# Ascend-Research/HeadPoseEstimation-WHENet

Measured on NVIDIA H100. Metric: head-crops/sec @224x224 bf16, higher is better.
Workload: dtype bf16

## Files before the change

headposeestimation-whenet_b200/build.py:

```python
from __future__ import annotations

import os
import subprocess
import sys

HERE = os.path.dirname(os.path.abspath(__file__))
CSRC = os.path.join(HERE, "csrc")
OBJ = os.path.join(CSRC, "obj")
LIB = os.path.join(HERE, "libwhenet_b200.so")
_SIMT_TC = ["kernels_simt.cuh", "kernels_tc.cuh"]
_ABI = os.path.join("..", "..", "include", "whenet_b200.h")
UNITS = {
    "whenet_api.cu": _SIMT_TC + ["api_error.h", "kernels_fused.cuh", "kernels_crop.cuh", "kernels_overlay.cuh", "hershey_simplex.inc", "yuv.cuh", "kernels_k2.cuh", "kernels_tc32.cuh", "kernels_dwse.cuh", "kernels_k1x.cuh", "jpeg_api.h", _ABI],
    "inst_k1_bf16.cu": _SIMT_TC + ["kernels_fused.cuh", "kernels_dwse.cuh", "kernels_k1x.cuh"],
    "inst_k1_f16.cu": _SIMT_TC + ["kernels_fused.cuh"],
    "inst_dwse.cu": _SIMT_TC + ["kernels_fused.cuh", "kernels_dwse.cuh"],
    "inst_pw.cu": _SIMT_TC + ["kernels_fused.cuh", "kernels_k2.cuh"],
    "inst_yolo.cu": _SIMT_TC + ["kernels_yolo.cuh", "yuv.cuh"],
    "inst_yolo32.cu": _SIMT_TC + ["kernels_yolo.cuh", "kernels_yolo32.cuh", "yuv.cuh"],
    "yolo_api.cu": _SIMT_TC + ["kernels_yolo.cuh", "kernels_yolo32.cuh", "yuv.cuh", "api_error.h", _ABI],
    "jpeg_api.cu": ["kernels_jpeg.cuh", "jpeg_api.h", "api_error.h", _ABI],
}
SOURCES = list(UNITS)
HEADERS = sorted({h for hs in UNITS.values() for h in hs})

NVCC_FLAGS = ["-O3", "-std=c++17", "-gencode", "arch=compute_90a,code=sm_90a", "-lineinfo", "-Xcompiler", "-fPIC,-ffp-contract=off"]


def _obj(src: str) -> str:
    return os.path.join(OBJ, os.path.splitext(src)[0] + ".o")


def _unit_stale(src: str) -> bool:
    o = _obj(src)
    if not os.path.exists(o):
        return True
    t = os.path.getmtime(o)
    deps = [os.path.join(CSRC, d) for d in [src] + UNITS[src]] + [os.path.abspath(__file__)]
    return any(os.path.exists(d) and os.path.getmtime(d) > t for d in deps)


def _stale() -> bool:
    if not os.path.exists(LIB):
        return True
    t = os.path.getmtime(LIB)
    deps = [os.path.join(CSRC, d) for d in SOURCES + HEADERS] + [os.path.abspath(__file__)]
    return any(os.path.exists(d) and os.path.getmtime(d) > t for d in deps)


def build_lib(force: bool = False, verbose: bool = False) -> str:
    if not force and not _stale():
        return LIB
    from concurrent.futures import ThreadPoolExecutor
    nvcc = os.environ.get("NVCC", "/usr/local/cuda/bin/nvcc")
    os.makedirs(OBJ, exist_ok=True)
    todo = [s for s in SOURCES if force or _unit_stale(s)]

    def compile_unit(src):
        cmd = [nvcc] + NVCC_FLAGS + (["-Xptxas=-v"] if verbose else []) + ["-c", "-o", _obj(src), os.path.join(CSRC, src)]
        if verbose:
            print(" ".join(cmd), file=sys.stderr)
        return src, subprocess.run(cmd, capture_output=True, text=True)

    with ThreadPoolExecutor(max_workers=max(1, min(len(todo), os.cpu_count() or 1))) as ex:
        results = list(ex.map(compile_unit, todo))
    for src, r in results:
        if r.returncode != 0:
            raise RuntimeError("nvcc failed on %s:\n%s\n%s" % (src, r.stdout, r.stderr))
        if verbose:
            print(r.stderr, file=sys.stderr)
# ... 10 lines not shown
```

headposeestimation-whenet_b200/csrc/inst_pw.cu:

```cuda
#include "kernels_simt.cuh"
#include "kernels_tc.cuh"
#include "kernels_k2.cuh"

namespace whenet {
namespace tc {
#define WHENET_INST_PW(T)                                                                                                    \
    template int launch_pw_tc2<T>(cudaStream_t, const T*, const void*, const float*, const float*, const T*, T*, long long, \
                                  int, int, int, bool, int, int, int, bool);                                                 \
    template int launch_k2<T>(cudaStream_t, const K2Params&, size_t, bool, bool, bool, int);                \
    template int launch_pw_tc3<T>(cudaStream_t, const T*, const void*, const float*, const float*, const T*, T*, long long, int, int, int);
WHENET_INST_PW(__nv_bfloat16)
WHENET_INST_PW(__half)
#undef WHENET_INST_PW
}
}
```

headposeestimation-whenet_b200/csrc/kernels_tc.cuh:

```cuda
#pragma once
#include <cuda.h>
#include <cuda_bf16.h>
#include <cuda_fp16.h>
#include <cuda_runtime.h>
#include <stdint.h>

#include "kernels_simt.cuh"

namespace whenet {
namespace tc {


constexpr int BM = 128;
constexpr int BK = 64;
constexpr int A_STAGE_BYTES = BM * BK * 2;
constexpr int kAccPitch = 132;
__host__ __device__ constexpr uint32_t acc_tile_bytes(int cols) { return (uint32_t)cols * kAccPitch * 4u; }

__device__ __forceinline__ uint32_t smem_u32(const void* p) { return (uint32_t)__cvta_generic_to_shared(p); }

__device__ __forceinline__ void mbar_init(uint64_t* bar, uint32_t count) {
    asm volatile("mbarrier.init.shared::cta.b64 [%0], %1;" ::"r"(smem_u32(bar)), "r"(count) : "memory");
}
__device__ __forceinline__ bool mbar_wait(uint64_t* bar, uint32_t parity, int* tflag) {
// ... 43 lines not shown
    if ((threadIdx.x & 31) == 0) arrive(bar_addr);
}
__device__ __forceinline__ void arrive_expect_tx(uint32_t bar_addr, uint32_t bytes) {
    asm volatile("mbarrier.arrive.expect_tx.shared::cta.b64 _, [%0], %1;" ::"r"(bar_addr), "r"(bytes) : "memory");
}
__device__ __forceinline__ void tma_4d(uint32_t dst, const CUtensorMap* tm, int c0, int c1, int c2, int c3, uint32_t bar_addr) {
    asm volatile("cp.async.bulk.tensor.4d.shared::cluster.global.mbarrier::complete_tx::bytes [%0], [%1, {%2, %3, %4, %5}], [%6];"
                 ::"r"(dst), "l"(tm), "r"(c0), "r"(c1), "r"(c2), "r"(c3), "r"(bar_addr) : "memory");
}
__device__ __forceinline__ void tma_2d(uint32_t dst, const CUtensorMap* tm, int c0, int c1, uint32_t bar_addr) {
    asm volatile("cp.async.bulk.tensor.2d.shared::cluster.global.mbarrier::complete_tx::bytes [%0], [%1, {%2, %3}], [%4];"
                 ::"r"(dst), "l"(tm), "r"(c0), "r"(c1), "r"(bar_addr) : "memory");
}

}

__device__ __forceinline__ uint64_t make_desc(uint32_t saddr) {
    uint64_t d = 0;
    d |= (uint64_t)((saddr >> 4) & 0x3FFF);
    d |= (uint64_t)1 << 16;
    d |= (uint64_t)64 << 32;
    d |= (uint64_t)1 << 62;
    return d;
}
__device__ __forceinline__ uint64_t make_desc_sw64(uint32_t saddr) {
    uint64_t d = 0;
    d |= (uint64_t)((saddr >> 4) & 0x3FFF);
    d |= (uint64_t)1 << 16;
    d |= (uint64_t)32 << 32;
    d |= (uint64_t)2 << 62;
    return d;
}
template <int ROWB>
__device__ __forceinline__ uint64_t make_desc_rows(uint32_t saddr) {
    static_assert(ROWB == 64 || ROWB == 128, "rows of 64 or 128 bytes");
    if constexpr (ROWB == 64) return make_desc_sw64(saddr);
    else return make_desc(saddr);
}

__device__ __forceinline__ void wg_fence() { asm volatile("wgmma.fence.sync.aligned;" ::: "memory"); }
__device__ __forceinline__ void wg_commit() { asm volatile("wgmma.commit_group.sync.aligned;" ::: "memory"); }
template <int N> __device__ __forceinline__ void wg_wait() { asm volatile("wgmma.wait_group.sync.aligned %0;" ::"n"(N) : "memory"); }

#define WG_D8(g) "+f"(d[8 * g]), "+f"(d[8 * g + 1]), "+f"(d[8 * g + 2]), "+f"(d[8 * g + 3]), \
                 "+f"(d[8 * g + 4]), "+f"(d[8 * g + 5]), "+f"(d[8 * g + 6]), "+f"(d[8 * g + 7])
#define WG_OPS_1 WG_D8(0)
#define WG_OPS_2 WG_OPS_1, WG_D8(1)
#define WG_OPS_3 WG_OPS_2, WG_D8(2)
#define WG_OPS_4 WG_OPS_3, WG_D8(3)
#define WG_OPS_5 WG_OPS_4, WG_D8(4)
#define WG_OPS_6 WG_OPS_5, WG_D8(5)
#define WG_OPS_7 WG_OPS_6, WG_D8(6)
#define WG_OPS_8 WG_OPS_7, WG_D8(7)
#define WG_REGS_1 "%0,%1,%2,%3,%4,%5,%6,%7"
#define WG_REGS_2 WG_REGS_1 ",%8,%9,%10,%11,%12,%13,%14,%15"
#define WG_REGS_3 WG_REGS_2 ",%16,%17,%18,%19,%20,%21,%22,%23"
#define WG_REGS_4 WG_REGS_3 ",%24,%25,%26,%27,%28,%29,%30,%31"
#define WG_REGS_5 WG_REGS_4 ",%32,%33,%34,%35,%36,%37,%38,%39"
#define WG_REGS_6 WG_REGS_5 ",%40,%41,%42,%43,%44,%45,%46,%47"
#define WG_REGS_7 WG_REGS_6 ",%48,%49,%50,%51,%52,%53,%54,%55"
#define WG_REGS_8 WG_REGS_7 ",%56,%57,%58,%59,%60,%61,%62,%63"
#define WG_TAIL_1 "16", "%8, %9", "%10"
#define WG_TAIL_2 "32", "%16, %17", "%18"
#define WG_TAIL_3 "48", "%24, %25", "%26"
#define WG_TAIL_4 "64", "%32, %33", "%34"
#define WG_TAIL_5 "80", "%40, %41", "%42"
#define WG_TAIL_6 "96", "%48, %49", "%50"
#define WG_TAIL_7 "112", "%56, %57", "%58"
#define WG_TAIL_8 "128", "%64, %65", "%66"
#define WG_ASM_(TY, REGS, NS, AB, SC, ...)                                                                              \
    asm volatile("{\n\t.reg .pred p;\n\tsetp.ne.b32 p, " SC ", 0;\n\t"                                                    \
                 "wgmma.mma_async.sync.aligned.m64n" NS "k16.f32." TY "." TY " {" REGS "}, " AB ", p, 1, 1, 0, 0;\n\t}" \
                 : __VA_ARGS__ : "l"(ad), "l"(bd), "r"(accumulate))
#define WG_ASM(TY, REGS, TAIL, OPS) WG_ASM_(TY, REGS, TAIL, OPS)
#define WG_CASE(k)                                                                                                 \
    if constexpr (N == 16 * k) {                                                                                   \
        if constexpr (BF16) WG_ASM("bf16", WG_REGS_##k, WG_TAIL_##k, WG_OPS_##k);                                  \
        else WG_ASM("f16", WG_REGS_##k, WG_TAIL_##k, WG_OPS_##k);                                                  \
    }

template <bool BF16, int N>
__device__ __forceinline__ void wgmma(float (&d)[N / 2], uint64_t ad, uint64_t bd, uint32_t accumulate) {
    static_assert(N % 16 == 0 && N >= 16 && N <= 128, "wgmma: N = 16, 32, ..., 128");
    WG_CASE(1) WG_CASE(2) WG_CASE(3) WG_CASE(4) WG_CASE(5) WG_CASE(6) WG_CASE(7) WG_CASE(8)
}
#undef WG_CASE
#undef WG_ASM
#undef WG_ASM_

template <int N> struct WgAcc { float d[2][N / 2]; };

template <bool BF16, int N, int H, int KS>
__device__ __forceinline__ void wg_mma_run(float (&d)[H][N / 2], uint64_t a0, uint64_t a1, uint64_t b0, uint32_t accumulate) {
    wg_fence();
#pragma unroll
    for (int k = 0; k < KS; ++k) {
        const uint32_t sc = (accumulate | (uint32_t)k) ? 1u : 0u;
        wgmma<BF16, N>(d[0], a0 + (uint64_t)(k * 2), b0 + (uint64_t)(k * 2), sc);
        if constexpr (H == 2) wgmma<BF16, N>(d[1], a1 + (uint64_t)(k * 2), b0 + (uint64_t)(k * 2), sc);
    }
    wg_commit();
}
template <bool BF16, int N, int H>
__device__ __forceinline__ void wg_mma_block(float (&d)[H][N / 2], uint64_t a0, uint64_t a1, uint64_t b0, int ksteps, uint32_t accumulate) {
    if (ksteps >= 4) wg_mma_run<BF16, N, H, 4>(d, a0, a1, b0, accumulate);
    else if (ksteps == 3) wg_mma_run<BF16, N, H, 3>(d, a0, a1, b0, accumulate);
    else if (ksteps == 2) wg_mma_run<BF16, N, H, 2>(d, a0, a1, b0, accumulate);
    else wg_mma_run<BF16, N, H, 1>(d, a0, a1, b0, accumulate);
}

template <bool BF16, int N>
__device__ __forceinline__ void wg_mma_tile(WgAcc<N>& acc, uint32_t a_st, uint32_t b_st, int ksteps, uint32_t accumulate) {
    wg_mma_block<BF16, N, 2>(acc.d, make_desc(a_st), make_desc(a_st + 64 * 128), make_desc(b_st), ksteps, accumulate);
}

template <bool BF16, int N>
__device__ __forceinline__ void wg_mma_m64(float (&d)[N / 2], uint32_t a_st, uint32_t a_kb, uint32_t b_st, uint32_t b_kb, int ksteps) {
    float (&d1)[1][N / 2] = *reinterpret_cast<float(*)[1][N / 2]>(&d);
    for (int kb = 0; kb * 4 < ksteps; ++kb)
        wg_mma_block<BF16, N, 1>(d1, make_desc(a_st + (uint32_t)kb * a_kb), 0, make_desc(b_st + (uint32_t)kb * b_kb), ksteps - 4 * kb, kb ? 1u : 0u);
}

template <int N>
__device__ __forceinline__ void wg_acc_store(const WgAcc<N>& acc, uint32_t dst, int wt) {
    const int w = wt >> 5, l = wt & 31;
    const int r = 16 * w + (l >> 2), cq = 2 * (l & 3);
#pragma unroll
    for (int h = 0; h < 2; ++h)
#pragma unroll
        for (int i = 0; i < N / 8; ++i)
#pragma unroll
            for (int e = 0; e < 4; ++e) {
                const int row = 64 * h + r + (e >> 1) * 8, col = 8 * i + cq + (e & 1);
                asm volatile("st.shared.f32 [%0], %1;" ::"r"(dst + (uint32_t)(col * kAccPitch + row) * 4u), "f"(acc.d[h][4 * i + e]) : "memory");
            }
}

// ... 24 lines not shown
        case 16: return call_with_width<16, MAXW>(f);
        case 32: return call_with_width<32, MAXW>(f);
        case 48: return call_with_width<48, MAXW>(f);
        case 64: return call_with_width<64, MAXW>(f);
        case 96: return call_with_width<96, MAXW>(f);
        case 128: return call_with_width<128, MAXW>(f);
    }
    return 1;
}

__device__ __forceinline__ void acc_ld16(uint32_t base, int row, int c0, float (&v)[16]) {
#pragma unroll
    for (int i = 0; i < 16; ++i)
        asm volatile("ld.shared.f32 %0, [%1];" : "=f"(v[i]) : "r"(base + (uint32_t)((c0 + i) * kAccPitch + row) * 4u));
}

template <typename T> __device__ __forceinline__ uint4 scale8(uint4 raw, const float* g);
template <> __device__ __forceinline__ uint4 scale8<__nv_bfloat16>(uint4 raw, const float* g) {
    __nv_bfloat162* h = reinterpret_cast<__nv_bfloat162*>(&raw);
    const float4 g0 = *reinterpret_cast<const float4*>(g), g1 = *reinterpret_cast<const float4*>(g + 4);
    const float gg[8] = {g0.x, g0.y, g0.z, g0.w, g1.x, g1.y, g1.z, g1.w};
#pragma unroll
    for (int i = 0; i < 4; ++i) {
        float2 f = __bfloat1622float2(h[i]);
        h[i] = __floats2bfloat162_rn(f.x * gg[2 * i], f.y * gg[2 * i + 1]);
    }
    return raw;
}
template <> __device__ __forceinline__ uint4 scale8<__half>(uint4 raw, const float* g) {
    __half2* h = reinterpret_cast<__half2*>(&raw);
    const float4 g0 = *reinterpret_cast<const float4*>(g), g1 = *reinterpret_cast<const float4*>(g + 4);
    const float gg[8] = {g0.x, g0.y, g0.z, g0.w, g1.x, g1.y, g1.z, g1.w};
#pragma unroll
    for (int i = 0; i < 4; ++i) {
        float2 f = __half22float2(h[i]);
        h[i] = __floats2half2_rn(f.x * gg[2 * i], f.y * gg[2 * i + 1]);
    }
    return raw;
}

__device__ __forceinline__ int fdiv_small(int x, float inv) { return __float2int_rz(((float)x + 0.5f) * inv); }
__device__ __forceinline__ void cp_async16_z(uint32_t dst, const void* src, bool valid) {
    const uint32_t sz = valid ? 16u : 0u;
    asm volatile("cp.async.cg.shared.global [%0], [%1], 16, %2;" ::"r"(dst), "l"(src), "r"(sz) : "memory");
}
__device__ __forceinline__ uint4 lds128(uint32_t addr) {
    uint4 v;
    asm volatile("ld.shared.v4.b32 {%0,%1,%2,%3}, [%4];" : "=r"(v.x), "=r"(v.y), "=r"(v.z), "=r"(v.w) : "r"(addr));
    return v;
}
__device__ __forceinline__ void sts128_(uint32_t addr, const uint4& v) {
    asm volatile("st.shared.v4.b32 [%0], {%1,%2,%3,%4};" ::"r"(addr), "r"(v.x), "r"(v.y), "r"(v.z), "r"(v.w) : "memory");
}
template <typename T> __device__ __forceinline__ uint4 scale8s(uint4 raw, uint32_t gaddr);
template <> __device__ __forceinline__ uint4 scale8s<__nv_bfloat16>(uint4 raw, uint32_t gaddr) {
    float4 g0, g1;
    asm volatile("ld.shared.v4.f32 {%0,%1,%2,%3}, [%4];" : "=f"(g0.x), "=f"(g0.y), "=f"(g0.z), "=f"(g0.w) : "r"(gaddr));
    asm volatile("ld.shared.v4.f32 {%0,%1,%2,%3}, [%4];" : "=f"(g1.x), "=f"(g1.y), "=f"(g1.z), "=f"(g1.w) : "r"(gaddr + 16));
    __nv_bfloat162* h = reinterpret_cast<__nv_bfloat162*>(&raw);
    const float gg[8] = {g0.x, g0.y, g0.z, g0.w, g1.x, g1.y, g1.z, g1.w};
#pragma unroll
    for (int i = 0; i < 4; ++i) {
        float2 f = __bfloat1622float2(h[i]);
        h[i] = __floats2bfloat162_rn(f.x * gg[2 * i], f.y * gg[2 * i + 1]);
    }
    return raw;
}
template <> __device__ __forceinline__ uint4 scale8s<__half>(uint4 raw, uint32_t gaddr) {
    float4 g0, g1;
    asm volatile("ld.shared.v4.f32 {%0,%1,%2,%3}, [%4];" : "=f"(g0.x), "=f"(g0.y), "=f"(g0.z), "=f"(g0.w) : "r"(gaddr));
    asm volatile("ld.shared.v4.f32 {%0,%1,%2,%3}, [%4];" : "=f"(g1.x), "=f"(g1.y), "=f"(g1.z), "=f"(g1.w) : "r"(gaddr + 16));
    __half2* h = reinterpret_cast<__half2*>(&raw);
    const float gg[8] = {g0.x, g0.y, g0.z, g0.w, g1.x, g1.y, g1.z, g1.w};
#pragma unroll
    for (int i = 0; i < 4; ++i) {
        float2 f = __half22float2(h[i]);
        h[i] = __floats2half2_rn(f.x * gg[2 * i], f.y * gg[2 * i + 1]);
    }
    return raw;
}

template <typename T, bool SWISH, int GATE, bool RESID, bool OUT_H, int UN>
__global__ void __launch_bounds__(128) pw_tc2_kernel(const T* __restrict__ A, const T* __restrict__ Wt,
                                                     const float* __restrict__ bias, const float* __restrict__ gate,
                                                     const T* __restrict__ resid, T* __restrict__ out,
                                                     int M, int K, int N, int hw,
                                                     int n_tile, int n_stages,
                                                     int tiles_per_crop) {
    constexpr bool BF16 = std::is_same<T, __nv_bfloat16>::value;
    extern __shared__ uint8_t smem_raw[];

    const int tid = threadIdx.x;
    const uint32_t smem0 = (smem_u32(smem_raw) + 1023u) & ~1023u;
    constexpr int w_stage_bytes = UN * BK * 2;
    const uint32_t stage_bytes = A_STAGE_BYTES + w_stage_bytes;
    const uint32_t sG = smem0 + n_stages * stage_bytes;

    int m0, rows_valid, crop0;
    if (GATE == 2) {
        const int crop = blockIdx.y / tiles_per_crop, t = blockIdx.y - crop * tiles_per_crop;
        m0 = crop * hw + t * BM;
        rows_valid = min(BM, hw - t * BM);
        crop0 = crop;
    } else {
        m0 = blockIdx.y * BM;
        rows_valid = min(BM, M - m0);
        crop0 = GATE ? m0 / hw : 0;
    }
    const int n0 = blockIdx.x * n_tile;
    const int n_valid = min(n_tile, N - n0);
    const int nkb = (K + BK - 1) / BK;
    const int kchunks = K >> 3;

    if (GATE) {
        const int ncrops = GATE == 2 ? 1 : ((m0 + rows_valid - 1) / hw - crop0 + 1);
        const int q = K >> 2;
        for (int idx = tid; idx < ncrops * q; idx += 128) {
            const int cr = idx / q, j = idx - cr * q;
            cp_async16_z(sG + (uint32_t)(cr * K + j * 4) * 4, gate + (long long)(crop0 + cr) * K + j * 4, true);
        }
    }
    auto fill = [&](int kb) {
        const int s = kb % n_stages;
        const uint32_t a_st = smem0 + s * stage_bytes, w_st = a_st + A_STAGE_BYTES;
        const int kc0 = kb * 8;
        const int cb = min(8, kchunks - kc0), cbp = (cb + 1) & ~1;
        if (cbp == 8) {
            const int c = tid & 7, r0 = tid >> 3;
            const bool cvalid = c < cb;
            const T* asrc = A + (long long)(m0 + r0) * K + (kc0 + c) * 8;
            const uint32_t swz = (uint32_t)((r0 >> 3) * 1024 + (r0 & 7) * 128 + ((c ^ (r0 & 7)) << 4));
#pragma unroll
// ... 371 lines not shown
```

headposeestimation-whenet_b200/csrc/whenet_api.cu:

```cuda
#include <cuda_bf16.h>
#include <cuda_fp16.h>
#include <cuda_runtime.h>

#include <algorithm>
#include <array>
#include <charconv>
#include <atomic>
#include <cmath>
#include <cstdarg>
#include <cstdio>
#include <cstdlib>
#include <cstring>
#include <map>
#include <string>
#include <thread>
#include <type_traits>
#include <vector>

#include "../../include/whenet_b200.h"
#include "api_error.h"
#include "kernels_simt.cuh"
#include "kernels_tc.cuh"
#include "kernels_fused.cuh"
#include "kernels_crop.cuh"
#include "kernels_overlay.cuh"
#include "kernels_k2.cuh"
#include "kernels_tc32.cuh"
#include "kernels_dwse.cuh"
#include "kernels_k1x.cuh"
#include "jpeg_api.h"
#include <cudaTypedefs.h>

namespace whenet {
namespace fused {
#define WHENET_EXTERN_FUSED(T)                                                                            \
    extern template int launch_k1<T>(cudaStream_t, K1Params, int, int, int, int, size_t, int);            \
    extern template int launch_dw_only<T>(cudaStream_t, K1Params, size_t, int);
WHENET_EXTERN_FUSED(__nv_bfloat16)
WHENET_EXTERN_FUSED(__half)
#undef WHENET_EXTERN_FUSED
extern template int launch_dwse<__nv_bfloat16>(cudaStream_t, DwSeParams, int, int, int, int, int);
extern template int launch_dwse_x<__nv_bfloat16>(cudaStream_t, DwSeParams, int, int, int, int, int);
extern template int launch_dwse_spatial<__nv_bfloat16>(cudaStream_t, DwSeParams, int, int, int);
extern template int launch_k1x<__nv_bfloat16>(cudaStream_t, DwSeParams, int, int, int, int, int, int, int, int);
}
namespace tc {
#define WHENET_EXTERN_PW(T)                                                                                                         \
    extern template int launch_pw_tc2<T>(cudaStream_t, const T*, const void*, const float*, const float*, const T*, T*, long long, \
                                         int, int, int, bool, int, int, int, bool);                                                 \
    extern template int launch_k2<T>(cudaStream_t, const K2Params&, size_t, bool, bool, bool, int);          \
    extern template int launch_pw_tc3<T>(cudaStream_t, const T*, const void*, const float*, const float*, const T*, T*, long long, int, int, int);
WHENET_EXTERN_PW(__nv_bfloat16)
WHENET_EXTERN_PW(__half)
#undef WHENET_EXTERN_PW
}
}

namespace {

using whenet::api::fail;
using whenet::api::g_err;

#define CK(call)                                                                                   \
    do {                                                                                           \
        cudaError_t e__ = (call);                                                                  \
        if (e__ != cudaSuccess)                                                                    \
            return fail(WHENET_ECUDA, "%s failed at %s:%d: %s", #call, __FILE__, __LINE__,         \
                        cudaGetErrorString(e__));                                                  \
    } while (0)

constexpr double kBnEps = 1e-3;
constexpr int kImgElems = 224 * 224 * 3;

struct BlockCfg {
    int idx, hin, hout, cin, cexp, cout, k, s, cse, pad;
    bool skip, has_expand;
};

std::vector<BlockCfg> make_blocks() {
// ... 307 lines not shown

int make_tmap_kd_e(CUtensorMap* tm, const void* base, int n, int H, int C, int cc, int pw) {
    auto fn = tmap_encode_fn();
    if (!fn) return fail(WHENET_ECUDA, "cuTensorMapEncodeTiled is not available from this driver");
    const cuuint64_t dims[4] = {(cuuint64_t)C, (cuuint64_t)H, (cuuint64_t)H, (cuuint64_t)n};
    const cuuint64_t strides[3] = {(cuuint64_t)C * 2, (cuuint64_t)H * C * 2, (cuuint64_t)H * H * C * 2};
    const cuuint32_t box[4] = {(cuuint32_t)cc, (cuuint32_t)pw, (cuuint32_t)pw, 1};
    const cuuint32_t estr[4] = {1, 1, 1, 1};
    const CUresult r = fn(tm, CU_TENSOR_MAP_DATA_TYPE_FLOAT16, 4, const_cast<void*>(base), dims, strides, box, estr, CU_TENSOR_MAP_INTERLEAVE_NONE,
                          CU_TENSOR_MAP_SWIZZLE_NONE, CU_TENSOR_MAP_L2_PROMOTION_L2_128B, CU_TENSOR_MAP_FLOAT_OOB_FILL_NONE);
    if (r != CUDA_SUCCESS) return fail(WHENET_ECUDA, "cuTensorMapEncodeTiled(KD tile %dx%dx%dx%d, box %dx%dx%d) failed: %d", n, H, H, C, pw, pw, cc, (int)r);
    return 0;
}
int make_tmap_k1x_in(CUtensorMap* tm, const void* base, int n, int H, int C, int iw, int row_bytes) {
    auto fn = tmap_encode_fn();
    if (!fn) return fail(WHENET_ECUDA, "cuTensorMapEncodeTiled is not available from this driver");
    const cuuint64_t dims[4] = {(cuuint64_t)C, (cuuint64_t)H, (cuuint64_t)H, (cuuint64_t)n};
    const cuuint64_t strides[3] = {(cuuint64_t)C * 2, (cuuint64_t)H * C * 2, (cuuint64_t)H * H * C * 2};
    const cuuint32_t box[4] = {(cuuint32_t)row_bytes / 2, (cuuint32_t)iw, (cuuint32_t)iw, 1};
    const cuuint32_t estr[4] = {1, 1, 1, 1};
    const CUresult r = fn(tm, CU_TENSOR_MAP_DATA_TYPE_BFLOAT16, 4, const_cast<void*>(base), dims, strides, box, estr, CU_TENSOR_MAP_INTERLEAVE_NONE,
                          row_bytes == 64 ? CU_TENSOR_MAP_SWIZZLE_64B : CU_TENSOR_MAP_SWIZZLE_128B, CU_TENSOR_MAP_L2_PROMOTION_L2_128B,
                          CU_TENSOR_MAP_FLOAT_OOB_FILL_NONE);
    if (r != CUDA_SUCCESS) return fail(WHENET_ECUDA, "cuTensorMapEncodeTiled(K1X input %dx%dx%dx%d, box %dx%d) failed: %d", n, H, H, C, iw, iw, (int)r);
    return 0;
}
int make_tmap_kd_w(CUtensorMap* tm, const void* base, int kk, int C, int cc) {
    auto fn = tmap_encode_fn();
    if (!fn) return fail(WHENET_ECUDA, "cuTensorMapEncodeTiled is not available from this driver");
    const cuuint64_t dims[2] = {(cuuint64_t)C, (cuuint64_t)kk};
    const cuuint64_t strides[1] = {(cuuint64_t)C * 2};
    const cuuint32_t box[2] = {(cuuint32_t)cc, (cuuint32_t)kk};
    const cuuint32_t estr[2] = {1, 1};
    const CUresult r = fn(tm, CU_TENSOR_MAP_DATA_TYPE_FLOAT16, 2, const_cast<void*>(base), dims, strides, box, estr, CU_TENSOR_MAP_INTERLEAVE_NONE,
                          CU_TENSOR_MAP_SWIZZLE_NONE, CU_TENSOR_MAP_L2_PROMOTION_L2_128B, CU_TENSOR_MAP_FLOAT_OOB_FILL_NONE);
    if (r != CUDA_SUCCESS) return fail(WHENET_ECUDA, "cuTensorMapEncodeTiled(KD weights %dx%d, box %d) failed: %d", kk, C, cc, (int)r);
    return 0;
}

template <typename T>
int launch_pw(whenet_ctx* c, const char* name, const T* A, const float* W, const void* Wt16, const float* bias,
              const float* gate, const T* resid, T* out, long long M, int K, int N, int hw, bool swish, bool out_half = false) {
    const double bytes = (double)M * (K + N + (resid ? N : 0)) * sizeof(T);
    const double flops = 2.0 * (double)M * K * N;
    Scope sc(c, name, bytes, flops);
    if constexpr (sizeof(T) == 2) {
        const bool want_k2 = c->pw_variant == 3 || (c->pw_variant == 4 && (gate == nullptr || hw <= 196));
        if (c->use_tc && Wt16 && want_k2 && !out_half) {
            whenet::tc::K2Params kp{};
            size_t smem = 0;
            if (whenet::tc::plan_k2(M, K, N, hw, gate != nullptr, c->precision == WHENET_PRECISION_BF16, &kp, &smem) &&
                (c->pw_variant == 3 || kp.tiles >= 2 * c->sm_count)) {
                if (c->tmaps2.size() > 1024) c->tmaps2.clear();
                const TmapKey ka{K, (int)M, (const void*)A}, kw{-N, K, Wt16};
                auto ia = c->tmaps2.find(ka);
                if (ia == c->tmaps2.end()) {
                    CUtensorMap tm;
                    int rc = make_tmap_w(&tm, A, (int)M, K, whenet::tc::BM, c->precision == WHENET_PRECISION_BF16);
                    if (rc) return rc;
                    ia = c->tmaps2.emplace(ka, tm).first;
                }
                auto iw = c->tmaps2.find(kw);
                if (iw == c->tmaps2.end()) {
                    CUtensorMap tm;
                    int rc = make_tmap_w(&tm, Wt16, N, K, kp.n_tile, c->precision == WHENET_PRECISION_BF16);
                    if (rc) return rc;
                    iw = c->tmaps2.emplace(kw, tm).first;
                }
                kp.tmA = ia->second; kp.tmW = iw->second;
                kp.bias = bias; kp.gate = gate; kp.resid = resid; kp.out = out; kp.tflag = c->d_tflag;
                int rc = whenet::tc::launch_k2<T>(c->stream, kp, smem, swish, gate != nullptr, resid != nullptr, c->sm_count);
                if (rc == 0) { CK(cudaGetLastError()); return 0; }
                if (rc < 0) return fail(WHENET_ECUDA, "K2 launch failed for %s (rc=%d)", name, rc);
            }
        }
        if (c->use_tc && Wt16 && gate && hw >= 784 && c->pw3 && !out_half && !swish) {
            int rc = whenet::tc::launch_pw_tc3<T>(c->stream, A, Wt16, bias, gate, resid, out, M, K, N, hw);
            if (rc == 0) { CK(cudaGetLastError()); return 0; }
            if (rc < 0) return fail(WHENET_ECUDA, "pw_tc3 launch failed for %s (rc=%d)", name, rc);
        }
        if (c->use_tc && Wt16) {
            int rc = whenet::tc::launch_pw_tc2<T>(c->stream, A, Wt16, bias, gate, resid, out, M, K, N, hw, swish, c->pw_stage_cap, c->pw_smem_kb, c->pw_min_ctas, out_half);
            if (rc == 0) { CK(cudaGetLastError()); return 0; }
            if (rc < 0) return fail(WHENET_ECUDA, "tensor-core 1x1 launch failed for %s (rc=%d)", name, rc);
        }
    }
    if constexpr (sizeof(T) == 4) {
        if (c->use_tc && Wt16 && c->split_lo_bytes) {
            int rc = whenet::tc::launch_pw_tc32(c->stream, A, Wt16, (const char*)Wt16 + c->split_lo_bytes, bias, gate, resid, out, M, K, N, hw, swish);
            if (rc == 0) { CK(cudaGetLastError()); return 0; }
            if (rc < 0) return fail(WHENET_ECUDA, "split-bf16 tensor-core 1x1 launch failed for %s (rc=%d)", name, rc);
        }
    }
    if (out_half) return fail(WHENET_EINVAL, "fp16-output 1x1 conv needs the tensor-core kernel (%s)", name);
    dim3 grid((unsigned)((M + 63) / 64), (unsigned)((N + 63) / 64));
#define PW(SW, GA, RE) whenet::pw_conv_kernel<T, SW, GA, RE><<<grid, 256, 0, c->stream>>>(A, W, bias, gate, resid, out, M, K, N, hw)
    if (swish && !gate && !resid) PW(true, false, false);
    else if (!swish && gate && !resid) PW(false, true, false);
    else if (!swish && gate && resid) PW(false, true, true);
    else if (!swish && !gate && !resid) PW(false, false, false);
    else if (!swish && !gate && resid) PW(false, false, true);
    else return fail(WHENET_EINVAL, "unsupported 1x1 epilogue combination");
#undef PW
    CK(cudaGetLastError());
    return 0;
}
// ... 1883 lines not shown
```

Measured before the change: 87470.

## Add crop-pair warp-specialized GEMM for gated 7x7 pointwise layers

Adds a persistent, warp-specialized wgmma kernel for bf16 pointwise convolutions at 7x7 spatial size (49 rows per crop) with N of 192 or 320. Each CTA processes two crops per tile so that TMA-loaded 49-row A tiles line up with crop boundaries. Gating warps apply the SE gate in shared memory between load and MMA, and the epilogue adds bias and optional residual through a shared-memory staging buffer. The wgmma helper is extended to N=160. The aim is to avoid wasted M padding and to fuse the gate scaling into the GEMM pipeline for the late network layers, at the cost of a new code path and a smaller M tile (98 rows) per CTA.

```diff
diff --git a/headposeestimation-whenet_b200/build.py b/headposeestimation-whenet_b200/build.py
--- a/headposeestimation-whenet_b200/build.py
+++ b/headposeestimation-whenet_b200/build.py
@@ -11,11 +11,11 @@
 _SIMT_TC = ["kernels_simt.cuh", "kernels_tc.cuh"]
 _ABI = os.path.join("..", "..", "include", "whenet_b200.h")
 UNITS = {
-    "whenet_api.cu": _SIMT_TC + ["api_error.h", "kernels_fused.cuh", "kernels_crop.cuh", "kernels_overlay.cuh", "hershey_simplex.inc", "yuv.cuh", "kernels_k2.cuh", "kernels_tc32.cuh", "kernels_dwse.cuh", "kernels_k1x.cuh", "jpeg_api.h", _ABI],
+    "whenet_api.cu": _SIMT_TC + ["api_error.h", "kernels_fused.cuh", "kernels_crop.cuh", "kernels_overlay.cuh", "hershey_simplex.inc", "yuv.cuh", "kernels_k2.cuh", "kernels_kp7.cuh", "kernels_tc32.cuh", "kernels_dwse.cuh", "kernels_k1x.cuh", "jpeg_api.h", _ABI],
     "inst_k1_bf16.cu": _SIMT_TC + ["kernels_fused.cuh", "kernels_dwse.cuh", "kernels_k1x.cuh"],
     "inst_k1_f16.cu": _SIMT_TC + ["kernels_fused.cuh"],
     "inst_dwse.cu": _SIMT_TC + ["kernels_fused.cuh", "kernels_dwse.cuh"],
-    "inst_pw.cu": _SIMT_TC + ["kernels_fused.cuh", "kernels_k2.cuh"],
+    "inst_pw.cu": _SIMT_TC + ["kernels_fused.cuh", "kernels_k2.cuh", "kernels_kp7.cuh"],
     "inst_yolo.cu": _SIMT_TC + ["kernels_yolo.cuh", "yuv.cuh"],
     "inst_yolo32.cu": _SIMT_TC + ["kernels_yolo.cuh", "kernels_yolo32.cuh", "yuv.cuh"],
     "yolo_api.cu": _SIMT_TC + ["kernels_yolo.cuh", "kernels_yolo32.cuh", "yuv.cuh", "api_error.h", _ABI],
diff --git a/headposeestimation-whenet_b200/csrc/inst_pw.cu b/headposeestimation-whenet_b200/csrc/inst_pw.cu
--- a/headposeestimation-whenet_b200/csrc/inst_pw.cu
+++ b/headposeestimation-whenet_b200/csrc/inst_pw.cu
@@ -1,6 +1,7 @@
 #include "kernels_simt.cuh"
 #include "kernels_tc.cuh"
 #include "kernels_k2.cuh"
+#include "kernels_kp7.cuh"
 
 namespace whenet {
 namespace tc {
@@ -12,5 +13,21 @@
 WHENET_INST_PW(__nv_bfloat16)
 WHENET_INST_PW(__half)
 #undef WHENET_INST_PW
+
+int launch_kp7(cudaStream_t stream, const KP7Params& p, size_t smem, bool resid) {
+    auto go = [&](auto kfn, int nt) {
+        if (cudaFuncSetAttribute(kfn, cudaFuncAttributeMaxDynamicSharedMemorySize, 225 * 1024) != cudaSuccess) return -1;
+        int dev = 0, sms = 0, per_sm = 0;
+        if (cudaGetDevice(&dev) != cudaSuccess || cudaDeviceGetAttribute(&sms, cudaDevAttrMultiProcessorCount, dev) != cudaSuccess ||
+            cudaOccupancyMaxActiveBlocksPerMultiprocessor(&per_sm, kfn, nt, smem) != cudaSuccess || per_sm < 1)
+            return -1;
+        kfn<<<(unsigned)std::min(p.pairs, per_sm * sms), nt, smem, stream>>>(p);
+        return 0;
+    };
+    if (p.N == 192 && resid) return go(kp7_kernel<192, true>, Kp7<192, true>::NT);
+    if (p.N == 192) return go(kp7_kernel<192, false>, Kp7<192, false>::NT);
+    if (p.N == 320 && !resid) return go(kp7_kernel<320, false>, Kp7<320, false>::NT);
+    return 1;
 }
 }
+}
diff --git a/headposeestimation-whenet_b200/csrc/kernels_kp7.cuh b/headposeestimation-whenet_b200/csrc/kernels_kp7.cuh
--- /dev/null
+++ b/headposeestimation-whenet_b200/csrc/kernels_kp7.cuh
@@ -0,0 +1,244 @@
+#pragma once
+#include <cuda.h>
+
+#include "kernels_fused.cuh"
+
+namespace whenet {
+namespace tc {
+
+constexpr int kKp7Hw = 49;
+constexpr uint32_t kKp7Half = 64 * 128;
+constexpr int kKp7GateThreads = 96;
+constexpr int kKp7MaxStages = 8;
+
+struct alignas(64) KP7Params {
+    CUtensorMap tmA;
+    CUtensorMap tmW;
+    const float* bias;
+    const float* gate;
+    const void* resid;
+    void* out;
+    int* tflag;
+    int K, N, crops, pairs;
+    int nkb, ksteps_last;
+    int stages;
+    uint32_t stage_bytes;
+    uint32_t off_g, off_b, off_o;
+};
+
+template <int N> struct Kp7Geom;
+template <> struct Kp7Geom<192> { static constexpr int NWG = 2, NW = 96; };
+template <> struct Kp7Geom<320> { static constexpr int NWG = 2, NW = 160; };
+
+template <int N, bool RESID>
+struct Kp7 {
+    static constexpr int NWG = Kp7Geom<N>::NWG, NW = Kp7Geom<N>::NW;
+    static constexpr int NT = 128 * (1 + NWG);
+    static constexpr int REG_LAUNCH = (65536 / NT) & ~7;
+    static constexpr int REG_LOW = 72;
+    static constexpr int REG_MMA = ((NT * REG_LAUNCH - 128 * REG_LOW) / (128 * NWG)) & ~7;
+    static constexpr uint32_t PITCH = RESID ? (uint32_t)(NW + 8) * 4u : (uint32_t)NW * 2u + 16u;
+    static constexpr uint32_t WARP_STAGE = 16u * PITCH;
+    static constexpr uint32_t OUT_STAGE = (uint32_t)(4 * NWG) * WARP_STAGE;
+    static_assert(NW % 16 == 0 && NW <= 160 && NW * NWG == N, "MMA width");
+    static_assert(REG_MMA >= NW + 24, "accumulator registers");
+};
+
+template <int N, bool RESID>
+__global__ void __launch_bounds__(Kp7<N, RESID>::NT, 1) kp7_kernel(const __grid_constant__ KP7Params p) {
+    using namespace whenet::fused;
+    using G = Kp7<N, RESID>;
+    constexpr int NW = G::NW;
+    extern __shared__ uint8_t smem_raw[];
+    __shared__ __align__(8) uint64_t bars[3 * kKp7MaxStages];
+    __shared__ int s_abort_mem;
+    volatile int* s_abort = &s_abort_mem;
+
+    const int tid = threadIdx.x, warp = tid >> 5, lane = tid & 31;
+    const uint32_t smem0 = (smem_u32(smem_raw) + 1023u) & ~1023u;
+    const uint32_t sRing = smem0, sG = smem0 + p.off_g, sB = smem0 + p.off_b;
+    const uint32_t bar0 = smem_u32(&bars[0]);
+    const uint32_t b_full = bar0, b_ready = bar0 + 8 * kKp7MaxStages, b_empty = bar0 + 16 * kKp7MaxStages;
+
+    if (tid == 0) {
+        for (int i = 0; i < kKp7MaxStages; ++i) {
+            mbar_init(&bars[i], 1);
+            mbar_init(&bars[kKp7MaxStages + i], kKp7GateThreads / 32);
+            mbar_init(&bars[2 * kKp7MaxStages + i], G::NWG);
+        }
+        s_abort_mem = 0;
+        asm volatile("fence.mbarrier_init.release.cluster;" ::: "memory");
+    }
+    for (int i = tid; i < N; i += G::NT) {
+        const float b = __ldg(p.bias + i);
+        asm volatile("st.shared.f32 [%0], %1;" ::"r"(sB + (uint32_t)i * 4u), "f"(b) : "memory");
+    }
+    __syncthreads();
+
+    const int first = blockIdx.x, step = gridDim.x;
+
+    if (warp < 4) {
+        asm volatile("setmaxnreg.dec.sync.aligned.u32 %0;" ::"n"(G::REG_LOW));
+        if (warp == 0) {
+            if (lane == 0) {
+                asm volatile("prefetch.tensormap [%0];" ::"l"(&p.tmA) : "memory");
+                asm volatile("prefetch.tensormap [%0];" ::"l"(&p.tmW) : "memory");
+                const uint32_t a_bytes = kKp7Hw * 128;
+                int g = 0;
+                for (int pair = first; pair < p.pairs; pair += step) {
+                    const bool two = 2 * pair + 1 < p.crops;
+                    const int row0 = 2 * pair * kKp7Hw;
+                    for (int kb = 0; kb < p.nkb; ++kb, ++g) {
+                        const int s = g % p.stages;
+                        const uint32_t par = (uint32_t)(g / p.stages) & 1u;
+                        mbar::wait(b_empty + 8 * s, par ^ 1, s_abort, p.tflag);
+                        const uint32_t st = sRing + (uint32_t)s * p.stage_bytes;
+                        mbar::arrive_expect_tx(b_full + 8 * s, (two ? 2 : 1) * a_bytes + (uint32_t)N * 128);
+                        mbar::tma_2d(st, &p.tmA, kb * 64, row0, b_full + 8 * s);
+                        if (two) mbar::tma_2d(st + kKp7Half, &p.tmA, kb * 64, row0 + kKp7Hw, b_full + 8 * s);
+#pragma unroll
+                        for (int j = 0; j < G::NWG; ++j)
+                            mbar::tma_2d(st + 2 * kKp7Half + (uint32_t)(j * NW * 128), &p.tmW, kb * 64, j * NW, b_full + 8 * s);
+                    }
+                }
+            }
+        } else {
+            const int gt = tid - 32;
+            const int c = gt & 7, r0 = gt >> 3;
+            const int kchunks = p.K >> 3;
+            int g = 0;
+            for (int pair = first; pair < p.pairs; pair += step) {
+                const int halves = 2 * pair + 1 < p.crops ? 2 : 1;
+                asm volatile("bar.sync 1, %0;" ::"n"(kKp7GateThreads) : "memory");
+                const int q = p.K >> 2;
+                const float4* grow = reinterpret_cast<const float4*>(p.gate + (long long)2 * pair * p.K);
+                for (int idx = gt; idx < halves * q; idx += kKp7GateThreads) cp_async16_z(sG + (uint32_t)idx * 16u, grow + idx, true);
+                asm volatile("cp.async.wait_all;" ::: "memory");
+                asm volatile("bar.sync 1, %0;" ::"n"(kKp7GateThreads) : "memory");
+                for (int kb = 0; kb < p.nkb; ++kb, ++g) {
+                    const int s = g % p.stages;
+                    const uint32_t par = (uint32_t)(g / p.stages) & 1u;
+                    mbar::wait(b_full + 8 * s, par, s_abort, p.tflag);
+                    const uint32_t st = sRing + (uint32_t)s * p.stage_bytes;
+                    if (kb * 8 + c < kchunks) {
+                        for (int h = 0; h < halves; ++h) {
+                            float4 g0, g1;
+                            lds_g8(sG + (uint32_t)(h * p.K + (kb * 8 + c) * 8) * 4u, g0, g1);
+                            const uint32_t a0 = st + (uint32_t)h * kKp7Half;
+                            uint4 v[5];
+#pragma unroll
+                            for (int i = 0; i < 5; ++i)
+                                if (r0 + 12 * i < kKp7Hw) v[i] = lds128(a0 + sw128(r0 + 12 * i, c));
+#pragma unroll
+                            for (int i = 0; i < 5; ++i)
+                                if (r0 + 12 * i < kKp7Hw) sts128_(a0 + sw128(r0 + 12 * i, c), scale8r<__nv_bfloat16>(v[i], g0, g1));
+                        }
+                    }
+                    asm volatile("fence.proxy.async.shared::cta;" ::: "memory");
+                    mbar::arrive_warp(b_ready + 8 * s);
+                }
+            }
+        }
+    } else {
+        asm volatile("setmaxnreg.inc.sync.aligned.u32 %0;" ::"n"(G::REG_MMA));
+        const int wg = (warp >> 2) - 1, wq = warp & 3, wt = tid & 127;
+        const int n0 = wg * NW;
+        const __nv_bfloat16* resid = reinterpret_cast<const __nv_bfloat16*>(p.resid);
+        __nv_bfloat16* out = reinterpret_cast<__nv_bfloat16*>(p.out);
+        const uint32_t sO = smem0 + p.off_o + (uint32_t)(warp - 4) * G::WARP_STAGE;
+        int g = 0;
+        for (int pair = first; pair < p.pairs; pair += step) {
+            WgAcc<NW> acc;
+            const int g0 = g;
+            for (int kb = 0; kb < p.nkb; ++kb, ++g) {
+                const int s = g % p.stages;
+                const uint32_t par = (uint32_t)(g / p.stages) & 1u;
+                mbar::wait(b_ready + 8 * s, par, s_abort, p.tflag);
+                const uint32_t a_st = sRing + (uint32_t)s * p.stage_bytes;
+                wg_mma_tile<true, NW>(acc, a_st, a_st + 2 * kKp7Half + (uint32_t)(n0 * 128), kb == p.nkb - 1 ? p.ksteps_last : 4, kb ? 1u : 0u);
+                if (kb > 0) {
+                    wg_wait<1>();
+                    asm volatile("bar.sync %0, 128;" ::"r"(2 + wg) : "memory");
+                    if (wt == 0) mbar::arrive(b_empty + 8 * ((g - 1) % p.stages));
+                }
+            }
+            wg_wait<0>();
+            asm volatile("bar.sync %0, 128;" ::"r"(2 + wg) : "memory");
+            if (wt == 0) mbar::arrive(b_empty + 8 * ((g0 + p.nkb - 1) % p.stages));
+            if (*s_abort) continue;
+            const int rows = min(16, kKp7Hw - 16 * wq);
+#pragma unroll
+            for (int h = 0; h < 2; ++h) {
+                const int crop = 2 * pair + h;
+                if (crop >= p.crops) continue;
+                __syncwarp();
+#pragma unroll
+                for (int e2 = 0; e2 < 2; ++e2) {
+                    const uint32_t srow = sO + (uint32_t)((lane >> 2) + 8 * e2) * G::PITCH;
+#pragma unroll
+                    for (int i = 0; i < NW / 8; ++i) {
+                        const int cl = 8 * i + 2 * (lane & 3);
+                        float2 b;
+                        asm volatile("ld.shared.v2.f32 {%0,%1}, [%2];" : "=f"(b.x), "=f"(b.y) : "r"(sB + (uint32_t)(n0 + cl) * 4u));
+                        const float o0 = acc.d[h][4 * i + 2 * e2] + b.x, o1 = acc.d[h][4 * i + 2 * e2 + 1] + b.y;
+                        if (RESID)
+                            asm volatile("st.shared.v2.f32 [%0], {%1,%2};" ::"r"(srow + (uint32_t)cl * 4u), "f"(o0), "f"(o1) : "memory");
+                        else
+                            asm volatile("st.shared.b32 [%0], %1;" ::"r"(srow + (uint32_t)cl * 2u), "r"(pack2<__nv_bfloat16>(o0, o1)) : "memory");
+                    }
+                }
+                __syncwarp();
+                constexpr int CPR = NW / 8;
+                const long long m0 = (long long)crop * kKp7Hw + 16 * wq;
+                int r = lane / CPR, j = lane - r * CPR;
+                for (; r < rows; r += 32 / CPR, j += 32 % CPR) {
+                    if (j >= CPR) { j -= CPR; ++r; if (r >= rows) break; }
+                    const long long off = (m0 + r) * N + n0 + 8 * j;
+                    uint4 v;
+                    if (RESID) {
+                        const uint32_t sa = sO + (uint32_t)r * G::PITCH + (uint32_t)j * 32u;
+                        const float4 x0 = lds_f4(sa), x1 = lds_f4(sa + 16);
+                        const uint4 rr = __ldg(reinterpret_cast<const uint4*>(resid + off));
+                        float r0, r1;
+                        unpack2<__nv_bfloat16>(rr.x, r0, r1); v.x = pack2<__nv_bfloat16>(x0.x + r0, x0.y + r1);
+                        unpack2<__nv_bfloat16>(rr.y, r0, r1); v.y = pack2<__nv_bfloat16>(x0.z + r0, x0.w + r1);
+                        unpack2<__nv_bfloat16>(rr.z, r0, r1); v.z = pack2<__nv_bfloat16>(x1.x + r0, x1.y + r1);
+                        unpack2<__nv_bfloat16>(rr.w, r0, r1); v.w = pack2<__nv_bfloat16>(x1.z + r0, x1.w + r1);
+                    } else {
+                        v = lds128(sO + (uint32_t)r * G::PITCH + (uint32_t)j * 16u);
+                    }
+                    *reinterpret_cast<uint4*>(out + off) = v;
+                }
+            }
+        }
+    }
+}
+
+inline bool plan_kp7(long long M, int K, int N, bool resid, KP7Params* p, size_t* smem_out) {
+    if ((N != 192 && N != 320) || (resid && N != 192) || (K & 7) || K < 64 || K > 1152 || M < 1 || M % kKp7Hw || M > 0x7fffffffLL) return false;
+    p->K = K; p->N = N;
+    p->crops = (int)(M / kKp7Hw);
+    p->pairs = (p->crops + 1) / 2;
+    p->nkb = (K + 63) / 64;
+    p->ksteps_last = ((K - (p->nkb - 1) * 64) + 15) / 16;
+    p->stage_bytes = 2 * kKp7Half + (uint32_t)N * 128;
+    const uint32_t o_stage = N == 320 ? Kp7<320, false>::OUT_STAGE : resid ? Kp7<192, true>::OUT_STAGE : Kp7<192, false>::OUT_STAGE;
+    const size_t fixed = (size_t)2 * K * 4 + (size_t)N * 4 + o_stage;
+    const size_t budget = 225 * 1024 - 1024;
+    int stages = kKp7MaxStages;
+    while (stages > 2 && (size_t)stages * p->stage_bytes + fixed > budget) --stages;
+    if ((size_t)stages * p->stage_bytes + fixed > budget) return false;
+    p->stages = stages;
+    p->off_g = (uint32_t)stages * p->stage_bytes;
+    p->off_b = p->off_g + (uint32_t)(2 * K * 4);
+    p->off_o = p->off_b + (uint32_t)((N * 4 + 15) & ~15);
+    *smem_out = (size_t)p->off_o + o_stage + 1024;
+    return true;
+}
+
+inline int kp7_mma_width(int N) { return N == 320 ? Kp7Geom<320>::NW : Kp7Geom<192>::NW; }
+
+int launch_kp7(cudaStream_t stream, const KP7Params& p, size_t smem, bool resid);
+
+}
+}
diff --git a/headposeestimation-whenet_b200/csrc/kernels_tc.cuh b/headposeestimation-whenet_b200/csrc/kernels_tc.cuh
--- a/headposeestimation-whenet_b200/csrc/kernels_tc.cuh
+++ b/headposeestimation-whenet_b200/csrc/kernels_tc.cuh
@@ -119,6 +119,8 @@
 #define WG_OPS_6 WG_OPS_5, WG_D8(5)
 #define WG_OPS_7 WG_OPS_6, WG_D8(6)
 #define WG_OPS_8 WG_OPS_7, WG_D8(7)
+#define WG_OPS_9 WG_OPS_8, WG_D8(8)
+#define WG_OPS_10 WG_OPS_9, WG_D8(9)
 #define WG_REGS_1 "%0,%1,%2,%3,%4,%5,%6,%7"
 #define WG_REGS_2 WG_REGS_1 ",%8,%9,%10,%11,%12,%13,%14,%15"
 #define WG_REGS_3 WG_REGS_2 ",%16,%17,%18,%19,%20,%21,%22,%23"
@@ -127,6 +129,8 @@
 #define WG_REGS_6 WG_REGS_5 ",%40,%41,%42,%43,%44,%45,%46,%47"
 #define WG_REGS_7 WG_REGS_6 ",%48,%49,%50,%51,%52,%53,%54,%55"
 #define WG_REGS_8 WG_REGS_7 ",%56,%57,%58,%59,%60,%61,%62,%63"
+#define WG_REGS_9 WG_REGS_8 ",%64,%65,%66,%67,%68,%69,%70,%71"
+#define WG_REGS_10 WG_REGS_9 ",%72,%73,%74,%75,%76,%77,%78,%79"
 #define WG_TAIL_1 "16", "%8, %9", "%10"
 #define WG_TAIL_2 "32", "%16, %17", "%18"
 #define WG_TAIL_3 "48", "%24, %25", "%26"
@@ -135,6 +139,8 @@
 #define WG_TAIL_6 "96", "%48, %49", "%50"
 #define WG_TAIL_7 "112", "%56, %57", "%58"
 #define WG_TAIL_8 "128", "%64, %65", "%66"
+#define WG_TAIL_9 "144", "%72, %73", "%74"
+#define WG_TAIL_10 "160", "%80, %81", "%82"
 #define WG_ASM_(TY, REGS, NS, AB, SC, ...)                                                                              \
     asm volatile("{\n\t.reg .pred p;\n\tsetp.ne.b32 p, " SC ", 0;\n\t"                                                    \
                  "wgmma.mma_async.sync.aligned.m64n" NS "k16.f32." TY "." TY " {" REGS "}, " AB ", p, 1, 1, 0, 0;\n\t}" \
@@ -148,8 +154,8 @@
 
 template <bool BF16, int N>
 __device__ __forceinline__ void wgmma(float (&d)[N / 2], uint64_t ad, uint64_t bd, uint32_t accumulate) {
-    static_assert(N % 16 == 0 && N >= 16 && N <= 128, "wgmma: N = 16, 32, ..., 128");
-    WG_CASE(1) WG_CASE(2) WG_CASE(3) WG_CASE(4) WG_CASE(5) WG_CASE(6) WG_CASE(7) WG_CASE(8)
+    static_assert(N % 16 == 0 && N >= 16 && N <= 160, "wgmma: N = 16, 32, ..., 160");
+    WG_CASE(1) WG_CASE(2) WG_CASE(3) WG_CASE(4) WG_CASE(5) WG_CASE(6) WG_CASE(7) WG_CASE(8) WG_CASE(9) WG_CASE(10)
 }
 #undef WG_CASE
 #undef WG_ASM
@@ -280,11 +286,8 @@
 __device__ __forceinline__ void sts128_(uint32_t addr, const uint4& v) {
     asm volatile("st.shared.v4.b32 [%0], {%1,%2,%3,%4};" ::"r"(addr), "r"(v.x), "r"(v.y), "r"(v.z), "r"(v.w) : "memory");
 }
-template <typename T> __device__ __forceinline__ uint4 scale8s(uint4 raw, uint32_t gaddr);
-template <> __device__ __forceinline__ uint4 scale8s<__nv_bfloat16>(uint4 raw, uint32_t gaddr) {
-    float4 g0, g1;
-    asm volatile("ld.shared.v4.f32 {%0,%1,%2,%3}, [%4];" : "=f"(g0.x), "=f"(g0.y), "=f"(g0.z), "=f"(g0.w) : "r"(gaddr));
-    asm volatile("ld.shared.v4.f32 {%0,%1,%2,%3}, [%4];" : "=f"(g1.x), "=f"(g1.y), "=f"(g1.z), "=f"(g1.w) : "r"(gaddr + 16));
+template <typename T> __device__ __forceinline__ uint4 scale8r(uint4 raw, const float4& g0, const float4& g1);
+template <> __device__ __forceinline__ uint4 scale8r<__nv_bfloat16>(uint4 raw, const float4& g0, const float4& g1) {
     __nv_bfloat162* h = reinterpret_cast<__nv_bfloat162*>(&raw);
     const float gg[8] = {g0.x, g0.y, g0.z, g0.w, g1.x, g1.y, g1.z, g1.w};
 #pragma unroll
@@ -294,10 +297,7 @@
     }
     return raw;
 }
-template <> __device__ __forceinline__ uint4 scale8s<__half>(uint4 raw, uint32_t gaddr) {
-    float4 g0, g1;
-    asm volatile("ld.shared.v4.f32 {%0,%1,%2,%3}, [%4];" : "=f"(g0.x), "=f"(g0.y), "=f"(g0.z), "=f"(g0.w) : "r"(gaddr));
-    asm volatile("ld.shared.v4.f32 {%0,%1,%2,%3}, [%4];" : "=f"(g1.x), "=f"(g1.y), "=f"(g1.z), "=f"(g1.w) : "r"(gaddr + 16));
+template <> __device__ __forceinline__ uint4 scale8r<__half>(uint4 raw, const float4& g0, const float4& g1) {
     __half2* h = reinterpret_cast<__half2*>(&raw);
     const float gg[8] = {g0.x, g0.y, g0.z, g0.w, g1.x, g1.y, g1.z, g1.w};
 #pragma unroll
@@ -306,6 +306,15 @@
         h[i] = __floats2half2_rn(f.x * gg[2 * i], f.y * gg[2 * i + 1]);
     }
     return raw;
+}
+__device__ __forceinline__ void lds_g8(uint32_t gaddr, float4& g0, float4& g1) {
+    asm volatile("ld.shared.v4.f32 {%0,%1,%2,%3}, [%4];" : "=f"(g0.x), "=f"(g0.y), "=f"(g0.z), "=f"(g0.w) : "r"(gaddr));
+    asm volatile("ld.shared.v4.f32 {%0,%1,%2,%3}, [%4];" : "=f"(g1.x), "=f"(g1.y), "=f"(g1.z), "=f"(g1.w) : "r"(gaddr + 16));
+}
+template <typename T> __device__ __forceinline__ uint4 scale8s(uint4 raw, uint32_t gaddr) {
+    float4 g0, g1;
+    lds_g8(gaddr, g0, g1);
+    return scale8r<T>(raw, g0, g1);
 }
 
 template <typename T, bool SWISH, int GATE, bool RESID, bool OUT_H, int UN>
diff --git a/headposeestimation-whenet_b200/csrc/whenet_api.cu b/headposeestimation-whenet_b200/csrc/whenet_api.cu
--- a/headposeestimation-whenet_b200/csrc/whenet_api.cu
+++ b/headposeestimation-whenet_b200/csrc/whenet_api.cu
@@ -25,6 +25,7 @@
 #include "kernels_crop.cuh"
 #include "kernels_overlay.cuh"
 #include "kernels_k2.cuh"
+#include "kernels_kp7.cuh"
 #include "kernels_tc32.cuh"
 #include "kernels_dwse.cuh"
 #include "kernels_k1x.cuh"
@@ -438,6 +439,31 @@
             if (whenet::tc::plan_k2(M, K, N, hw, gate != nullptr, c->precision == WHENET_PRECISION_BF16, &kp, &smem) &&
                 (c->pw_variant == 3 || kp.tiles >= 2 * c->sm_count)) {
                 if (c->tmaps2.size() > 1024) c->tmaps2.clear();
+                if constexpr (std::is_same<T, __nv_bfloat16>::value) {
+                    whenet::tc::KP7Params q{};
+                    size_t qsmem = 0;
+                    if (c->pw_variant == 4 && gate && hw == whenet::tc::kKp7Hw && !swish &&
+                        whenet::tc::plan_kp7(M, K, N, resid != nullptr, &q, &qsmem)) {
+                        const TmapKey qa{K, -(int)M, (const void*)A}, qw{-N, -K, Wt16};
+                        auto ia = c->tmaps2.find(qa);
+                        if (ia == c->tmaps2.end()) {
+                            CUtensorMap tm;
+                            if (int rc = make_tmap_w(&tm, A, (int)M, K, whenet::tc::kKp7Hw, true)) return rc;
+                            ia = c->tmaps2.emplace(qa, tm).first;
+                        }
+                        auto iw = c->tmaps2.find(qw);
+                        if (iw == c->tmaps2.end()) {
+                            CUtensorMap tm;
+                            if (int rc = make_tmap_w(&tm, Wt16, N, K, whenet::tc::kp7_mma_width(N), true)) return rc;
+                            iw = c->tmaps2.emplace(qw, tm).first;
+                        }
+                        q.tmA = ia->second; q.tmW = iw->second;
+                        q.bias = bias; q.gate = gate; q.resid = resid; q.out = out; q.tflag = c->d_tflag;
+                        int rc = whenet::tc::launch_kp7(c->stream, q, qsmem, resid != nullptr);
+                        if (rc == 0) { CK(cudaGetLastError()); return 0; }
+                        if (rc < 0) return fail(WHENET_ECUDA, "KP7 launch failed for %s (rc=%d)", name, rc);
+                    }
+                }
                 const TmapKey ka{K, (int)M, (const void*)A}, kw{-N, K, Wt16};
                 auto ia = c->tmaps2.find(ka);
                 if (ia == c->tmaps2.end()) {
```

Measured after the change: 90530 (median of 6 runs). 3.5% higher.
